# likojack/ODAM

Measured on AMD Instinct MI355X. Metric: frames/sec end-to-end (DETR detect + SQ fit), 640x480 ScanNet, 1/2/4/8 GPU, higher is better.
Workload: dtype f32

## Files before the change

include/odam_detr.h:

```cpp
#ifndef ODAM_DETR_H
#define ODAM_DETR_H
#ifdef __cplusplus
extern "C" {
#endif

typedef struct odam_detr odam_detr;

typedef struct {
    int resnet_blocks[4];
    int hidden_dim;
    int nheads;
    int dim_feedforward;
    int enc_layers;
    int dec_layers;
    int num_queries;
    int num_classes1;
    int angle_bins;
    int max_batch;
    int img_h, img_w;
    int dtype;
    int pre_norm;
    int dilation;
    int basic_block;
} odam_detr_cfg;
// ... 35 lines not shown
int odam_op_conv2d_nhwc(const float* x, const float* w_packed, const float* scale, const float* bias,
                        const float* residual, float* y, int B, int H, int W, int Cin, int Cout, int KH, int KW,
                        int stride, int pad, int Kpad, int relu, int k_order, void* stream);
int odam_op_conv2d_nhwc_bf16(const void* x, const void* w_packed, const float* scale, const float* bias,
                             const void* residual, void* y, int B, int H, int W, int Cin, int Cout, int KH, int KW,
                             int stride, int pad, int Kpad, int relu, int out_f32, int k_order, void* stream);
int odam_op_conv2d_nhwc_ex(const void* x, const void* w_packed, const float* scale, const float* bias, const void* residual,
                           void* y, int B, int H, int W, int Cin, int Cout, int KH, int KW, int stride, int pad, int dil,
                           int Kpad, int relu, int k_order, int dtype, int out_f32, void* stream);
int odam_op_bottleneck_bf16(const void* x, const void* w2, const float* s2, const float* b2, const void* w3, const float* s3,
                            const float* b3, const void* residual, void* y, const void* w1n, const float* s1n, const float* b1n,
                            void* y_next, int B, int H, int W, int P, int stride, int PN, void* stream);
int odam_op_bottleneck_f32(const float* x, const float* w2, const float* s2, const float* b2, const float* w3, const float* s3,
                           const float* b3, const float* residual, float* y, const float* w1n, const float* s1n, const float* b1n,
                           float* y_next, int B, int H, int W, int P, int stride, int PN, void* stream);
long long odam_op_conv_paths(char* buf, int n, int reset);
int odam_op_conv_bf16_mode(int mode);
int odam_op_conv_f32_mode(int mode);
long long odam_op_pooled_stem_launches(void);
int odam_op_attention(const float* Q, int ldq, const float* K, int ldk, const float* V, int ldv, float* O, int ldo,
                      int B, int H, int Lq, int Lk, void* stream);
int odam_op_attention_bf16(const void* Q, int ldq, const void* K, int ldk, const void* V, int ldv, void* O, int ldo,
                           int B, int H, int Lq, int Lk, void* stream);
int odam_op_add_layernorm(const float* x, const float* r, const float* gamma, const float* beta, float* y, int M,
                          void* stream);
int odam_op_attention_ex(const void* Q, int ldq, const void* K, int ldk, const void* V, int ldv, void* O, int ldo,
                         int B, int H, int Lq, int Lk, int head_dim, int dtype, const unsigned char* key_mask, void* stream);
int odam_op_add_layernorm_ex(const void* x, const void* r, const float* gamma, const float* beta, void* y,
                             const float* pos, int L, void* y_pos, int M, int dtype, void* stream);
int odam_op_quantize_mxfp8(const void* x, int src_dtype, long long n, void* q, void* s, void* stream);
int odam_op_dequantize_mxfp8(const void* q, const void* s, long long n, float* y, void* stream);
int odam_op_conv2d_nhwc_mxfp8(const void* x, const void* xs, const void* w_packed, const void* ws, const float* scale,
                              const float* bias, const void* residual, void* y, void* ys, void* y_bf16, float* y_f32,
                              int B, int H, int W, int Cin, int Cout, int KH, int KW, int stride, int pad, int dil,
// ... 8 lines not shown
```

odam_amd/csrc/cg_big.hpp:

```cpp
#pragma once
#include "cg_common.hpp"
#include "cg_tails_f32.hpp"
#include "cg_tail_bf16.hpp"
#include "cg_launch.h"

namespace odam_cg {

constexpr int big_bm(int BN, int NTH) { return (NTH == 1024 && BN == 64) ? 512 : 256; }
constexpr int big_wm(int MODE, int BN, int NTH) {
    return NTH == 1024 ? (BN == 64 ? 16 : 4)
         : MODE >= 3 ? (BN == 256 ? ((MODE == 4 && CG_X16_WM8) ? 8 : 4) : 8) : (BN == 256 ? 2 : (BN == 128 ? 4 : 8));
}
#ifndef CG_DEEP_A
#define CG_DEEP_A 1
#endif

constexpr bool big_deep_a(int MODE, int BN, int NST, int NTH) { return CG_DEEP_A != 0 && MODE == 0 && BN == 256 && NST == 4 && NTH == 1024; }
template <int MODE, int BN, int NST, int NTH>
constexpr int big_lds_bytes() {
    const int bm = big_bm(BN, NTH);
    const int ring = NST * (MODE >= 3 ? bm * 64 + 96 * BN : (bm + BN) * 64);
    const int wm = big_wm(MODE, BN, NTH);
    const int wn = NTH / 64 / wm;
    const int slab = MODE == 4 ? (NTH / 64) * 16 * ((BN / wn > 128 ? 128 : BN / wn) + 4) * 4 : (NTH / 64) * 32 * (BN / wn) * 4;
    const int s1 = (MODE == 0 && NTH == 512) ? (BN == 256 ? 2 : (BN == 128 ? 3 : 4)) * (384 * 64 + 3 * BN * 64) : 0;
    const int m = ring > slab ? ring : slab;
    const int deep = big_deep_a(MODE, BN, NST, NTH) ? (6 + 4) * 256 * 64 : 0;
    const int m2 = m > s1 ? m : s1;
    return m2 > deep ? m2 : deep;
}

template <int MODE, int BN, int NST, int NTH = 512, int FUSE = 0>
__global__ __launch_bounds__(NTH, (NTH == 1024 ? 4 : 2)) void conv_gemm_big_kernel(ConvGemmArgs a) {
    static_assert(!FUSE || (FUSE <= 4 && (MODE == 3 || MODE == 4) && NTH == 512 && ((FUSE != 3 && BN == 64) || (FUSE == 3 && BN == 128))) ||
                      (FUSE >= 5 && FUSE <= 8 && MODE == 0 && NTH == 512 && NST == 4),
                  "fused layers: pre-split filters with 64-column tiles (FUSE 1, 2, 4) or 128-column tiles (FUSE 3); bf16 (FUSE 5 + "
                  "log2(PN / 32), 5 = no chained reduce)");
    static_assert(MODE == 0 || MODE == 2 || MODE == 3 || MODE == 4,
                  "bf16 operands, fp32 split, fp32 split with pre-split filters (3: 32x32x16 matrix instruction, 4: 16x16x32)");
    static_assert(MODE != 4 || FUSE <= 4, "the 16x16x32 schedule: its own epilogue, or the fp32 bottleneck tails");
    constexpr bool BF16 = MODE == 0;
    constexpr bool PRE = MODE == 3 || MODE == 4;
    constexpr bool X16 = MODE == 4;
    static_assert(!PRE || NTH == 512 || (X16 && NTH == 1024), "pre-split filters: eight-wave workgroups, or sixteen waves (16x16x32 loop)");
    static_assert(NTH != 1024 || (FUSE == 0 && ((BN == 64 && (X16 || BF16)) || (BN == 256 && BF16))), "sixteen waves: plain layers (512 x 64: bf16 or the 16x16x32 split loop; 256 x 256: bf16)");
    using T = typename std::conditional<BF16, unsigned short, float>::type;
    constexpr int EPC = BF16 ? 8 : 4;
    constexpr int BM = big_bm(BN, NTH), BKE = 4 * EPC;
    constexpr int KU = 2 * BKE;
    constexpr int NW = NTH / 64;
    constexpr int WM = big_wm(MODE, BN, NTH), WN = NW / WM;
    constexpr int TM = BM / WM / 32, TN = BN / WN / 32;
    constexpr int RPP = NTH / 4;
    constexpr int A_LD = BM / RPP, B_LD = (BN + RPP - 1) / RPP;
    constexpr int ROWB = 64;
// ... 450 lines not shown
            for (int i = 0; i < MI; i++)
#pragma unroll
                for (int j = 0; j < NJ; j++) asm volatile("" :: "v"(c16[i][j]));
#if CG_HACK & 2
#pragma unroll
            for (int i = 0; i < 8; i++) asm volatile("" :: "v"(hk_l[i]));
#endif
            return;
        }
#endif
        if constexpr (FUSE != 0 || POOLABLE) __syncthreads();
        if constexpr (FUSE == 1) { fused_second(a, c16, smem, lds_base, m0, wave, lane); return; }
        if constexpr (FUSE == 2) { fused_chain(a, c16, smem, lds_base, m0, wave, lane); return; }
        if constexpr (FUSE == 3) { fused_second128(a, c16, smem, lds_base, m0, wave, lane); return; }
        if constexpr (FUSE == 4) { fused_chain128(a, c16, smem, lds_base, m0, wave, lane); return; }
        if constexpr (POOLABLE) {
            if (a.pool) {
                constexpr int SLD = BN + 4;
                static_assert(BM * SLD * 4 <= NST * STAGE, "the pooling slab fits the ring");
                float* S = smem;
                float scv[NJ], biv[NJ];
#pragma unroll
                for (int j = 0; j < NJ; j++) {
                    const int n = j * 16 + r16;
                    scv[j] = a.scale ? a.scale[n] : 1.0f; biv[j] = a.bias ? a.bias[n] : 0.0f;
                }
#pragma unroll
                for (int mi = 0; mi < MI; mi++)
#pragma unroll
                    for (int r = 0; r < 4; r++) {
// ... 450 lines not shown
                    const int n = wn * (BN / WN) + j * 32 + l32;
                    const float sc = a.scale ? a.scale[n] : 1.0f, bi = a.bias ? a.bias[n] : 0.0f;
#pragma unroll
                    for (int r = 0; r < 16; r++) {
                        const int R = wm * (BM / WM) + i * 32 + (r & 3) + 8 * (r >> 2) + 4 * half;
                        float v = acc[i][j][r] * sc + bi;
                        v = bf2f(f2bf(v));
                        S[R * SLD + n] = (pool_row_ok(R) && v > 0.f) ? v : 0.f;
                    }
                }
            __syncthreads();
            pool_store(S);
            return;
        }
    }
    if constexpr (FUSE >= 5) {
        fused_bf16<BN, FUSE == 5 ? 0 : (32 << (FUSE - 5)), FUSE == 7 ? 2 : 3>(a, acc, smem, lds_base, m0, wm, wn, wave, lane);
        return;
    }
    static_assert(X16 || (WM * WN * 32 * (BN / WN) * 4 <= big_lds_bytes<MODE, BN, NST, NTH>() && NST * STAGE <= big_lds_bytes<MODE, BN, NST, NTH>()),
                  "ring and epilogue staging fit the dynamic LDS");
    if (ep2) epilogue2<BM, BN, WM, WN, TM, TN, BF16>(a, acc, smem, m0, n0, wm, wn, wave, lane);
    else epilogue<BM, BN, WM, WN, TM, TN, BF16>(a, acc, smem, big_lds_bytes<MODE, BN, NST, NTH>() / 4, m0, n0, wm, wn, wave, lane);
}

#define g_s1_window odam_cfg::get(odam_cfg::CG_S1)

template <int MODE, int BN, int NST, int NTH = 512>
static int launch_big(const ConvGemmArgs& a_in, hipStream_t stream) {
    ConvGemmArgs a = a_in;
    a.s1_window = (MODE == 0 && NTH == 512) ? g_s1_window : 0;
// ... 21 lines not shown
```

odam_amd/csrc/cg_fused_f32.hip:

```cpp
#include "cg_big.hpp"

#include <algorithm>

namespace odam_cg {

template <int MODE>
static int launch_big_fused_as(const ConvGemmArgs& a, hipStream_t stream) {
    static const bool attr_ok = [] {
        return hipFuncSetAttribute((const void*)conv_gemm_big_kernel<MODE, 64, 4, 512, 1>, hipFuncAttributeMaxDynamicSharedMemorySize, FUSE_LDS_BYTES) == hipSuccess &&
               hipFuncSetAttribute((const void*)conv_gemm_big_kernel<MODE, 64, 4, 512, 2>, hipFuncAttributeMaxDynamicSharedMemorySize, FUSE_LDS_BYTES) == hipSuccess &&
               hipFuncSetAttribute((const void*)conv_gemm_big_kernel<MODE, 128, 4, 512, 3>, hipFuncAttributeMaxDynamicSharedMemorySize, FUSE_LDS_BYTES) == hipSuccess &&
               hipFuncSetAttribute((const void*)conv_gemm_big_kernel<MODE, 64, 4, 512, 4>, hipFuncAttributeMaxDynamicSharedMemorySize, FUSE_LDS_BYTES) == hipSuccess;
    }();
    if (!attr_ok) return odam_fail(2, "conv_gemm: cannot raise the dynamic LDS limit");
    const int tiles = (a.M + 255) / 256;
    if (a.Cout == 128) hipLaunchKernelGGL((conv_gemm_big_kernel<MODE, 128, 4, 512, 3>), dim3(tiles), dim3(512), FUSE_LDS_BYTES, stream, a);
    else if (a.G_Wt3 && a.G_N == 128) hipLaunchKernelGGL((conv_gemm_big_kernel<MODE, 64, 4, 512, 4>), dim3(tiles), dim3(512), FUSE_LDS_BYTES, stream, a);
    else if (a.G_Wt3) hipLaunchKernelGGL((conv_gemm_big_kernel<MODE, 64, 4, 512, 2>), dim3(tiles), dim3(512), FUSE_LDS_BYTES, stream, a);
    else hipLaunchKernelGGL((conv_gemm_big_kernel<MODE, 64, 4, 512, 1>), dim3(tiles), dim3(512), FUSE_LDS_BYTES, stream, a);
    ODAM_HIP(hipGetLastError());
    return 0;
}
int launch_big_fused(const ConvGemmArgs& a, hipStream_t stream) {
    const int m16 = odam_cfg::get(odam_cfg::CG_MFMA16);
    const bool x16 = a.Kpad % 32 == 0 && (m16 >= 3 || (m16 == 2 && a.Cout == 128));
    note_path("f32.fused.m%d.%s", x16 ? 4 : 3, a.Cout == 128 ? "l2" : !a.G_Wt3 ? "l1" : a.G_N == 128 ? "chain128" : "chain64");
    const long img_rows = (long)a.Ho * a.Wo, img_bytes = img_rows * a.F_ldc * 4;
    const int group = (int)std::min<long>(a.B, (0x7fffffffL - 1) / img_bytes);
    if (group < 1) return odam_fail(1, "conv_gemm: fused bottleneck: one image's output exceeds 2 GiB");
    const long lda = a.lda > 0 ? a.lda : a.Cin;
    for (int b0 = 0; b0 < a.B; b0 += group) {
        ConvGemmArgs g = a;
        g.B = std::min(group, a.B - b0);
        g.M = (int)(g.B * img_rows);
        g.A = reinterpret_cast<const float*>(a.A) + (size_t)b0 * a.H * a.W * lda;
        if (a.F_res) g.F_res = a.F_res + (size_t)b0 * img_rows * a.F_ldc;
        g.F_C = a.F_C + (size_t)b0 * img_rows * a.F_ldc;
        if (a.G_C) g.G_C = a.G_C + (size_t)b0 * img_rows * a.G_N;
        const int rc = x16 ? launch_big_fused_as<4>(g, stream) : launch_big_fused_as<3>(g, stream);
        if (rc) return rc;
    }
    return 0;
}

}

#if CG_STAMP
extern "C" int odam_cg_tail_stamps(unsigned long long* out8, int reset) {
    if (out8 && hipMemcpyFromSymbol(out8, HIP_SYMBOL(odam_cg::g_tail_stamps), 8 * sizeof(unsigned long long)) != hipSuccess) return 2;
    if (reset) {
        unsigned long long z[8] = {0, 0, 0, 0, 0, 0, 0, 0};
// ... 6 lines not shown
```

odam_amd/csrc/cg_tails_f32.hpp:

```cpp
#pragma once
#include "cg_common.hpp"

namespace odam_cg {

template <class ACC>
__device__ __forceinline__ void fused_second(const ConvGemmArgs& a, ACC& acc, float* smem, unsigned lds_base,
                                             int m0, int wave, int lane) {
    typedef __bf16 bf16x8 __attribute__((ext_vector_type(8)));
    const int half = lane >> 5, l32 = lane & 31;
    const int wave_u = __builtin_amdgcn_readfirstlane(wave);
    const TailAffine t1(a.scale, a.bias, a.relu, a.Cout), tF(a.F_scale, a.F_bias, a.F_relu, a.F_ldc);
    float sc1[4], bi1[4];
    cols64_affine(acc, t1, 0, lane, sc1, bi1);
    {
        const unsigned long long pf = (unsigned long long)a.F_Wt3;
        const u32x4 rs = u32x4{(unsigned)pf, (unsigned)(pf >> 32) & 0xffffu, OOB_VOFF, 0x00020000u};
#pragma unroll
        for (int j = 0; j < 12; j++) {
            const int q = wave_u + 8 * j;
            const int sp = q >> 3, rb = q & 7, s_ = sp / 3, pl = sp - 3 * s_;
            const int row = rb * 32 + (lane >> 1);
            const unsigned vo = (unsigned)(row * 384 + s_ * 96 + pl * 32 + (((lane & 1) ^ ((lane >> 4) & 1)) * 16));
            lds_dma16(rs, lds_base + (unsigned)(q * 1024), vo, 0);
        }
// ... 229 lines not shown
    wave_sync();
#pragma unroll
    for (int it = 0; it < 8; it++) {
        const int row = it * 4 + (lane >> 4);
        const int m = m_base + row;
        const float4 v = *reinterpret_cast<const float4*>(&slab[row * 64 + ((c4 ^ (row & 15)) << 2)]);
        if (m < a.M) *reinterpret_cast<float4*>(a.G_C + (size_t)m * 64 + c4 * 4) = v;
    }
#if CG_STAMP
    CG_TSTAMP(7);
    if (lane == 0) {
        for (int i = 0; i < 8; i++) if (i != 5) atomicAdd(&g_tail_stamps[i], ts_acc[i]);
        atomicAdd(&g_tail_stamps[5], 1ull);
    }
#endif
}

template <class ACC>
__device__ __forceinline__ void fused_chain128(const ConvGemmArgs& a, ACC& acc, float* smem, unsigned lds_base,
                                               int m0, int wave, int lane) {
    typedef __bf16 bf16x8 __attribute__((ext_vector_type(8)));
    constexpr int SLABS = 8 * 32 * 64 * 4, GB = 4 * 3 * 64 * 32, GB2 = 4 * 3 * 128 * 32;
    static_assert(SLABS + 2 * GB + GB2 == 160 * 1024, "slabs, two expand groups and one reduce slice fill the LDS");
    int half = lane >> 5, l32 = lane & 31;
    const int wave_u = __builtin_amdgcn_readfirstlane(wave);
    const TailAffine t1(a.scale, a.bias, a.relu, a.Cout), tF(a.F_scale, a.F_bias, a.F_relu, a.F_ldc);
    float sc1[4], bi1[4];
    cols64_affine(acc, t1, 0, lane, sc1, bi1);
    const unsigned long long pf = (unsigned long long)a.F_Wt3, pg = (unsigned long long)a.G_Wt3;
    const u32x4 rsf = u32x4{(unsigned)pf, (unsigned)(pf >> 32) & 0xffffu, OOB_VOFF, 0x00020000u};
// ... 286 lines not shown
```

odam_amd/csrc/conv_gemm.h:

```cpp
#pragma once
#include <hip/hip_runtime.h>
#include <stdint.h>

namespace odam_cg {

constexpr int ODAM_CG_F32 = 0;
constexpr int ODAM_CG_BF16 = 1;

struct ConvGemmArgs {
    const void* A;
    const void* Wt;
    const void* Wt3 = nullptr;
    const float* scale;
    const float* bias;
    const void* res;
    void* C;
    int B, H, W, Cin, log2Cin;
    int Ho, Wo, Cout;
    int KH, KW, stride, pad;
    int Kpad;
    int relu;
    int M;
    int ldc;
    int dtype;
    int out_f32;
    int lda;
    int k_order;
    const void* F_Wt3 = nullptr;
    const float* F_scale = nullptr;
    const float* F_bias = nullptr;
    const float* F_res = nullptr;
    float* F_C = nullptr;
    int F_ldc = 0, F_relu = 0;
    const void* G_Wt3 = nullptr;
    const float* G_scale = nullptr;
    const float* G_bias = nullptr;
    float* G_C = nullptr;
    int G_N = 64;
    const void* F_Wt = nullptr;
    const void* G_Wt = nullptr;
    int dil = 1;
    int pool = 0, pool_ph = 0, pool_pw = 0, Hp = 0, Wp = 0;
    int no_pin = 0;
    int s1_window = 0;
};

constexpr int POOL_PH = 8, POOL_PW = 14;

int launch_conv_gemm(const ConvGemmArgs& a, hipStream_t stream);

void set_big_mode(int mode);

void set_f32_mode(int mode);
// ... 15 lines not shown
```

odam_amd/csrc/conv_gemm.hip:

```cpp
#include "conv_gemm.h"

#include "cg_common.hpp"
#include "cg_launch.h"

#include <algorithm>
#include <cstdarg>
#include <cstdio>
#include <mutex>

namespace odam_cg {

static std::mutex g_path_mu;
static char g_path_ring[PATH_LOG_N][PATH_TOKEN_LEN];
static long long g_path_head = 0, g_path_base = 0;

void note_path(const char* fmt, ...) {
    char tok[PATH_TOKEN_LEN];
    va_list ap;
    va_start(ap, fmt);
    vsnprintf(tok, sizeof(tok), fmt, ap);
    va_end(ap);
    std::lock_guard<std::mutex> lk(g_path_mu);
    memcpy(g_path_ring[g_path_head % PATH_LOG_N], tok, sizeof(tok));
    g_path_head++;
// ... 377 lines not shown
    const bool x3 = !bf && ut && g_big_f32 == 2 && odam_cfg::get(odam_cfg::CG_SMALL_X3) != 0;
    note_path("%s.small.%dx%d.w%d%s%s%s", bf ? "bf16" : "f32", BM, BN, WM * WN, ut ? ".ut" : "", x3 ? ".x3" : "", ut && NST_UT == 4 ? ".s4" : "");
    if (bf) {
        if (ut) hipLaunchKernelGGL((conv_gemm_kernel<BM, BN, WM, WN, true, true, NST_UT>), g, b, 0, stream, a);
        else hipLaunchKernelGGL((conv_gemm_kernel<BM, BN, WM, WN, true, false>), g, b, 0, stream, a);
    } else {
        if (x3)
            hipLaunchKernelGGL((conv_gemm_kernel<BM, BN, WM, WN, false, true, NST_UT, true>), g, b, 0, stream, a);
        else if (ut) hipLaunchKernelGGL((conv_gemm_kernel<BM, BN, WM, WN, false, true, NST_UT>), g, b, 0, stream, a);
        else hipLaunchKernelGGL((conv_gemm_kernel<BM, BN, WM, WN, false, false>), g, b, 0, stream, a);
    }
    ODAM_HIP(hipGetLastError());
    return 0;
}

bool fused_second_ok(const ConvGemmArgs& a) {
    const int fuse = odam_cfg::get(odam_cfg::CG_FUSE);
    if (!fuse || !g_big_mode || g_big_f32 != 2 || a.dtype != ODAM_CG_F32) return false;
    if (!a.F_Wt3 || !a.F_C || !a.Wt3 || a.Kpad % 16 != 0) return false;
    const bool l1 = a.Cout == 64 && a.F_ldc == 256, l2 = a.Cout == 128 && a.F_ldc == 512 && !a.G_Wt3;
    if ((!l1 && !l2) || a.dil != 1) return false;
    if ((long)a.Cout * a.Kpad * 6 >= 0x7fffffffL || (long)a.Ho * a.Wo * a.F_ldc * 4 >= 0x7fffffffL) return false;
    if (a.G_Wt3 && (fuse < 2 || !a.G_C || (a.G_N != 64 && a.G_N != 128))) return false;
    return big_eligible(a, a.Cout);
}

#define g_fuse_bf16 odam_cfg::get(odam_cfg::CG_FUSE_BF16)
bool fused_bf16_ok(const ConvGemmArgs& a) {
    if (!g_fuse_bf16 || !g_big_mode || a.dtype != ODAM_CG_BF16 || !a.F_Wt || !a.F_C) return false;
    if (a.Cout != 64 && a.Cout != 128 && a.Cout != 256) return false;
    if (a.F_ldc != 4 * a.Cout || a.KH * a.KW != 9 || a.Cin != a.Cout || !a.k_order || a.dil != 1) return false;
    if ((long)a.M * a.F_ldc * 2 >= 0x7fffffffL) return false;
    if (a.G_Wt) {
        if (g_fuse_bf16 < 2 || !a.G_C) return false;
        const bool built = (a.Cout == 64 && (a.G_N == 64 || a.G_N == 128)) || (a.Cout == 128 && a.G_N == 128);
        if (!built) return false;
    }
    return big_eligible(a, a.Cout);
// ... 76 lines not shown
```

odam_amd/csrc/detr_model.hip:

```cpp
#include <hip/hip_runtime.h>
#include <atomic>

#include <algorithm>
#include <cmath>
#include <cstdlib>
#include <cstring>
#include <map>
#include <string>
#include <vector>

#include "../../include/odam_detr.h"
#include "cg_mx8.h"
#include "conv_gemm.h"
#include "detr_kernels.h"
#include "odam_config.h"
#include "odam_err.h"

using odam_cg::ConvGemmArgs;

namespace {

struct HostTensor {
    std::vector<long long> shape;
    std::vector<float> data;
// ... 243 lines not shown
            hipEvent_t e;
            ODAM_HIP(hipEventCreate(&e));
            m->ev.push_back(e);
        }
        m->ev_flops.resize(m->ev.size() / 2);
    }
    const int Ho = conv_out(H, (c.KH - 1) * c.dil + 1, c.stride, c.pad), Wo = conv_out(W, (c.KW - 1) * c.dil + 1, c.stride, c.pad);
    const int Cin_true = (c.KH == 7) ? 3 : c.Cin;
    m->ev_flops[m->ev_used / 2] = 2.0 * B * Ho * Wo * (double)c.Cout * c.KH * c.KW * Cin_true;
    ODAM_HIP(hipEventRecord(m->ev[m->ev_used], st));
    int rc = run_conv(c, x, B, H, W, res, relu, y, 0, st, m->dt, out_f32);
    ODAM_HIP(hipEventRecord(m->ev[m->ev_used + 1], st));
    m->ev_used += 2;
    return rc;
}
int fused_c2c3_t(odam_detr* m, const Conv& c2, const Conv& c3, const void* x, int B, int H, int W, const void* res, void* y,
                 hipStream_t st, const Conv* next_c1 = nullptr, void* t_next = nullptr, bool* chained = nullptr) {
    if (chained) *chained = false;
    if (m->basic) return -1;
    if (c2.dil != 1) return -1;
    if (c3.KH != 1 || c3.stride != 1 || c3.Kpad != c2.Cout) return -1;
    if (!m->dt && (!c2.w3 || !c3.w3)) return -1;
    ConvGemmArgs a{};
    a.dtype = m->dt; a.out_f32 = 0;
    a.A = x; a.Wt = c2.w; a.Wt3 = c2.w3; a.scale = c2.scale; a.bias = c2.bias; a.res = nullptr; a.C = nullptr;
    a.B = B; a.H = H; a.W = W; a.Cin = c2.Cin; a.log2Cin = ilog2(c2.Cin);
    a.Ho = conv_out(H, c2.KH, c2.stride, c2.pad); a.Wo = conv_out(W, c2.KW, c2.stride, c2.pad);
    a.Cout = c2.Cout; a.KH = c2.KH; a.KW = c2.KW; a.stride = c2.stride; a.pad = c2.pad; a.Kpad = c2.Kpad;
    a.relu = 1; a.M = B * a.Ho * a.Wo; a.ldc = c2.Cout; a.k_order = c2.k_order;
    a.F_scale = c3.scale; a.F_bias = c3.bias; a.F_res = (const float*)res; a.F_C = (float*)y;
    a.F_ldc = c3.Cout; a.F_relu = 1;
    double flops3 = 0.0;
// ... 11 lines not shown
        }
        if (!odam_cg::fused_bf16_ok(a)) return -1;
    } else {
    a.F_Wt3 = c3.w3;
    if (next_ok && next_c1->w3 && (next_c1->Cout == 64 || next_c1->Cout == 128) && c3.Cout == 256) {
        a.G_Wt3 = next_c1->w3; a.G_scale = next_c1->scale; a.G_bias = next_c1->bias; a.G_C = (float*)t_next; a.G_N = next_c1->Cout;
        if (odam_cg::fused_second_ok(a)) {
            if (chained) *chained = true;
            flops3 = 2.0 * a.M * (double)next_c1->Cout * c3.Cout;
        } else {
            a.G_Wt3 = nullptr; a.G_scale = a.G_bias = nullptr; a.G_C = nullptr; a.G_N = 64;
        }
    }
    if (!odam_cg::fused_second_ok(a)) return -1;
    }
    if (!m->profile) return odam_cg::launch_conv_gemm(a, st);
    if (m->ev_used + 2 > m->ev.size()) {
        for (int k = 0; k < 2; k++) {
            hipEvent_t e;
            ODAM_HIP(hipEventCreate(&e));
            m->ev.push_back(e);
        }
        m->ev_flops.resize(m->ev.size() / 2);
    }
    m->ev_flops[m->ev_used / 2] = 2.0 * a.M * ((double)c2.Cout * c2.KH * c2.KW * c2.Cin + (double)c3.Cout * c2.Cout) + flops3;
    ODAM_HIP(hipEventRecord(m->ev[m->ev_used], st));
    int rc = odam_cg::launch_conv_gemm(a, st);
    ODAM_HIP(hipEventRecord(m->ev[m->ev_used + 1], st));
    m->ev_used += 2;
    return rc;
}

static std::atomic<long long> g_pooled_stem_launches{0};
int stem_rows_t(odam_detr* m, int B, hipStream_t st, void* pooled_out = nullptr, bool* pooled = nullptr) {
    const Conv& c = m->stem_rows;
    const odam_detr_cfg& g = m->cfg;
    ConvGemmArgs a{};
    a.dtype = m->dt; a.out_f32 = 0;
    a.A = m->x4; a.Wt = c.w; a.Wt3 = c.w3; a.scale = c.scale; a.bias = c.bias; a.res = nullptr; a.C = m->stem_out;
    a.B = B; a.H = g.img_h + 6; a.W = g.img_w + 8; a.Cin = 32; a.log2Cin = 5; a.lda = 4;
// ... 386 lines not shown
            RC(conv_t(m, b.ds, cur, B, H, W, nullptr, false, m->dsb, st));
            res = m->dsb;
        }
        RC(conv_t(m, b.c2, tin, B, Ho, Wo, res, true, nxt, st));
        char* t = cur; cur = nxt; nxt = t;
        H = Ho; W = Wo;
    }
    for (size_t i = 0; !m->mx && !m->basic && i < m->blocks.size(); i++) {
        mark(i);
        const Bottleneck& b = m->blocks[i];
        const int s = m->block_stride[i];
        const int Ho = conv_out(H, 3, s, 1), Wo = conv_out(W, 3, s, 1);
        if (!have_c1) RC(conv_t(m, b.c1, cur, B, H, W, nullptr, true, tin, st));
        have_c1 = false;
        const char* res = cur;
        if (b.has_ds) {
            RC(conv_t(m, b.ds, cur, B, H, W, nullptr, false, m->dsb, st));
            res = m->dsb;
        }
        const Conv* next_c1 = (i + 1 < m->blocks.size()) ? &m->blocks[i + 1].c1 : nullptr;
        bool chained = false;
        const int frc = fused_c2c3_t(m, b.c2, b.c3, tin, B, H, W, res, nxt, st, next_c1, tout, &chained);
        if (frc > 0) return frc;
        if (frc < 0) {
            RC(conv_t(m, b.c2, tin, B, H, W, nullptr, true, tout, st));
            RC(conv_t(m, b.c3, tout, B, Ho, Wo, res, true, nxt, st));
        } else if (chained) {
            char* t = tin; tin = tout; tout = t;
            have_c1 = true;
        }
        char* t = cur; cur = nxt; nxt = t;
        H = Ho; W = Wo;
    }
    m->layer4 = cur;
    m->stage_ev[5] = m->ev_used;
    const int L = m->L, M = B * L, Mq = B * Q;

    RC(conv_t(m, m->input_proj, cur, B, H, W, nullptr, false, m->src, st));
    const float* pos = pos_b ? pos_b : m->pos;
// ... 231 lines not shown
    if (!odam_cg::fused_second_ok(a)) return odam_fail(4, "odam_op_bottleneck_f32: the fused kernel does not apply to this shape");
    unsigned short *d2 = nullptr, *d3 = nullptr, *d1 = nullptr;
    int rc = split_filters_for_call(w2, P, 9 * P, st, &d2, "odam_op_bottleneck_f32");
    if (!rc) rc = split_filters_for_call(w3, 4 * P, P, st, &d3, "odam_op_bottleneck_f32");
    if (!rc && PN > 0) rc = split_filters_for_call(w1n, PN, 4 * P, st, &d1, "odam_op_bottleneck_f32");
    if (!rc) {
        a.Wt3 = d2; a.F_Wt3 = d3; a.G_Wt3 = PN > 0 ? d1 : nullptr;
        rc = odam_cg::launch_conv_gemm(a, st);
    }
    (void)hipStreamSynchronize(st);
    if (d2) (void)hipFree(d2);
    if (d3) (void)hipFree(d3);
    if (d1) (void)hipFree(d1);
    return rc;
}

extern "C" long long odam_op_conv_paths(char* buf, int n, int reset) { return odam_cg::read_paths(buf, n, reset); }

extern "C" int odam_op_conv_bf16_mode(int mode) {
    if (mode < 0 || mode > 2) return odam_fail(1, "odam_op_conv_bf16_mode: mode must be 0, 1 or 2");
    odam_cg::set_big_mode(mode);
    return 0;
}

extern "C" int odam_op_conv_f32_mode(int mode) {
    if (mode != 0 && mode != 2) return odam_fail(1, "odam_op_conv_f32_mode: mode must be 0 or 2");
    odam_cg::set_f32_mode(mode);
    return 0;
}

// ... 219 lines not shown
```

odam_amd/csrc/odam_common.hip:

```cpp
#include <atomic>
#include <cstdio>
#include <cstring>

#include "odam_config.h"
#include "odam_err.h"

extern "C" const char* odam_last_error(void) { return g_odam_err; }

namespace odam_cfg {
namespace {
struct Entry { const char* name; int def, lo, hi; };
const Entry TABLE[N_KEYS] = {
    {"cg.ring", 1, 0, 2},        {"cg.f32", 2, 0, 2},         {"cg.fuse", 2, 0, 2},       {"cg.fuse_bf16", 2, 0, 2},
    {"cg.s1", 1, 0, 1},          {"cg.ut", 1, 0, 1},          {"cg.tiles", 31, 0, 31},      {"cg.force", 0, 0, 3},
    {"cg.presplit", 1, 0, 1},    {"cg.mfma16", 3, 0, 3},      {"att.x3", 1, 0, 1},         {"att.bf16_mfma", 1, 0, 1}, {"stem.rows", 1, 0, 1},
    {"assoc.persist", 2, 0, 2},  {"sq.split", 32, 1, 32},     {"sq.split_wait", 3000, 0, 100000000}, {"sq.lanes", 0, 0, 64},
    {"stem.pool", 1, 0, 1},
    {"cg.pin", 0, 0, 1},
    {"cg.small_x3", 1, 0, 1},
    {"assoc.sk_fast", 1, 0, 3},
    {"assoc.hungarian", 0, 0, 1},
    {"assoc.merge", 1, 0, 1},
    {"sq.two_per_cu", 1, 0, 1},
};
std::atomic<int> g_val[N_KEYS];
std::atomic<bool> g_init{false};
void init() {
    if (g_init.load(std::memory_order_acquire)) return;
    for (int k = 0; k < N_KEYS; k++) g_val[k].store(TABLE[k].def, std::memory_order_relaxed);
    g_init.store(true, std::memory_order_release);
}
}
int get(Key k) { init(); return g_val[k].load(std::memory_order_relaxed); }
void set(Key k, int v) { init(); g_val[k].store(v, std::memory_order_relaxed); }
}

extern "C" int odam_config_set(const char* key, int value) {
    using namespace odam_cfg;
// ... 37 lines not shown
```

odam_amd/csrc/odam_config.h:

```cpp
#pragma once

namespace odam_cfg {
enum Key {
    CG_RING,
    CG_F32,
    CG_FUSE,
    CG_FUSE_BF16,
    CG_S1,
    CG_UT,
    CG_TILES,
    CG_FORCE,
    CG_PRESPLIT,
    CG_MFMA16,
    ATT_X3,
    ATT_BF16_MFMA,
    STEM_ROWS,
    ASSOC_PERSIST,
    SQ_SPLIT,
    SQ_SPLIT_WAIT,
    SQ_LANES,
    STEM_POOL,
    CG_PIN,
    CG_SMALL_X3,
    ASSOC_SK_FAST,
    ASSOC_HUNGARIAN,
    ASSOC_MERGE,
    SQ_TWO_PER_CU,
    N_KEYS
};
int get(Key k);
void set(Key k, int v);
}
```

Before: 1149.

## Fold the bottleneck downsample 1x1 conv into the fused c2/c3 tile kernel

Adds a FUSE=9 variant of the fp32 pre-split 16x16x32 conv-GEMM that computes the downsample 1x1 projection of the block input on the same tile and uses it as the residual for the c3 epilogue. This drops a separate downsample launch and the write/read of the dsb intermediate for the first block of layer1 (stride 1, 64 channels). It adds LDS pressure, extra MFMA work per tile and more register use, and falls back to the old path when the shape or config does not fit. The new path is controlled by the cg.fuse_ds key, which is on by default.

```diff
diff --git a/include/odam_detr.h b/include/odam_detr.h
--- a/include/odam_detr.h
+++ b/include/odam_detr.h
@@ -73,10 +73,15 @@
 int odam_op_bottleneck_f32(const float* x, const float* w2, const float* s2, const float* b2, const float* w3, const float* s3,
                            const float* b3, const float* residual, float* y, const float* w1n, const float* s1n, const float* b1n,
                            float* y_next, int B, int H, int W, int P, int stride, int PN, void* stream);
+int odam_op_bottleneck_ds_f32(const float* x, const float* w2, const float* s2, const float* b2, const float* w3, const float* s3,
+                              const float* b3, const float* xin, const float* wd, const float* sd, const float* bd, float* y,
+                              const float* w1n, const float* s1n, const float* b1n, float* y_next, int B, int H, int W, int P,
+                              int stride, int PN, void* stream);
 long long odam_op_conv_paths(char* buf, int n, int reset);
 int odam_op_conv_bf16_mode(int mode);
 int odam_op_conv_f32_mode(int mode);
 long long odam_op_pooled_stem_launches(void);
+long long odam_op_fused_ds_launches(void);
 int odam_op_attention(const float* Q, int ldq, const float* K, int ldk, const float* V, int ldv, float* O, int ldo,
                       int B, int H, int Lq, int Lk, void* stream);
 int odam_op_attention_bf16(const void* Q, int ldq, const void* K, int ldk, const void* V, int ldv, void* O, int ldo,
diff --git a/odam_amd/csrc/cg_big.hpp b/odam_amd/csrc/cg_big.hpp
--- a/odam_amd/csrc/cg_big.hpp
+++ b/odam_amd/csrc/cg_big.hpp
@@ -33,12 +33,12 @@
 template <int MODE, int BN, int NST, int NTH = 512, int FUSE = 0>
 __global__ __launch_bounds__(NTH, (NTH == 1024 ? 4 : 2)) void conv_gemm_big_kernel(ConvGemmArgs a) {
     static_assert(!FUSE || (FUSE <= 4 && (MODE == 3 || MODE == 4) && NTH == 512 && ((FUSE != 3 && BN == 64) || (FUSE == 3 && BN == 128))) ||
-                      (FUSE >= 5 && FUSE <= 8 && MODE == 0 && NTH == 512 && NST == 4),
+                      (FUSE >= 5 && FUSE <= 8 && MODE == 0 && NTH == 512 && NST == 4) || (FUSE == 9 && MODE == 4 && NTH == 512 && BN == 64),
                   "fused layers: pre-split filters with 64-column tiles (FUSE 1, 2, 4) or 128-column tiles (FUSE 3); bf16 (FUSE 5 + "
-                  "log2(PN / 32), 5 = no chained reduce)");
+                  "log2(PN / 32), 5 = no chained reduce); FUSE 9 = FUSE 2 with the downsample on the tile (16x16x32 loop)");
     static_assert(MODE == 0 || MODE == 2 || MODE == 3 || MODE == 4,
                   "bf16 operands, fp32 split, fp32 split with pre-split filters (3: 32x32x16 matrix instruction, 4: 16x16x32)");
-    static_assert(MODE != 4 || FUSE <= 4, "the 16x16x32 schedule: its own epilogue, or the fp32 bottleneck tails");
+    static_assert(MODE != 4 || FUSE <= 4 || FUSE == 9, "the 16x16x32 schedule: its own epilogue, or the fp32 bottleneck tails");
     constexpr bool BF16 = MODE == 0;
     constexpr bool PRE = MODE == 3 || MODE == 4;
     constexpr bool X16 = MODE == 4;
@@ -519,6 +519,7 @@
         if constexpr (FUSE == 2) { fused_chain(a, c16, smem, lds_base, m0, wave, lane); return; }
         if constexpr (FUSE == 3) { fused_second128(a, c16, smem, lds_base, m0, wave, lane); return; }
         if constexpr (FUSE == 4) { fused_chain128(a, c16, smem, lds_base, m0, wave, lane); return; }
+        if constexpr (FUSE == 9) { fused_chain_ds(a, c16, smem, lds_base, m0, wave, lane); return; }
         if constexpr (POOLABLE) {
             if (a.pool) {
                 constexpr int SLD = BN + 4;
@@ -999,7 +1000,7 @@
             return;
         }
     }
-    if constexpr (FUSE >= 5) {
+    if constexpr (FUSE >= 5 && FUSE <= 8) {
         fused_bf16<BN, FUSE == 5 ? 0 : (32 << (FUSE - 5)), FUSE == 7 ? 2 : 3>(a, acc, smem, lds_base, m0, wm, wn, wave, lane);
         return;
     }
diff --git a/odam_amd/csrc/cg_fused_f32.hip b/odam_amd/csrc/cg_fused_f32.hip
--- a/odam_amd/csrc/cg_fused_f32.hip
+++ b/odam_amd/csrc/cg_fused_f32.hip
@@ -10,11 +10,15 @@
         return hipFuncSetAttribute((const void*)conv_gemm_big_kernel<MODE, 64, 4, 512, 1>, hipFuncAttributeMaxDynamicSharedMemorySize, FUSE_LDS_BYTES) == hipSuccess &&
                hipFuncSetAttribute((const void*)conv_gemm_big_kernel<MODE, 64, 4, 512, 2>, hipFuncAttributeMaxDynamicSharedMemorySize, FUSE_LDS_BYTES) == hipSuccess &&
                hipFuncSetAttribute((const void*)conv_gemm_big_kernel<MODE, 128, 4, 512, 3>, hipFuncAttributeMaxDynamicSharedMemorySize, FUSE_LDS_BYTES) == hipSuccess &&
-               hipFuncSetAttribute((const void*)conv_gemm_big_kernel<MODE, 64, 4, 512, 4>, hipFuncAttributeMaxDynamicSharedMemorySize, FUSE_LDS_BYTES) == hipSuccess;
+               hipFuncSetAttribute((const void*)conv_gemm_big_kernel<MODE, 64, 4, 512, 4>, hipFuncAttributeMaxDynamicSharedMemorySize, FUSE_LDS_BYTES) == hipSuccess &&
+               (MODE != 4 || hipFuncSetAttribute((const void*)conv_gemm_big_kernel<4, 64, 4, 512, 9>, hipFuncAttributeMaxDynamicSharedMemorySize, FUSE_LDS_BYTES) == hipSuccess);
     }();
     if (!attr_ok) return odam_fail(2, "conv_gemm: cannot raise the dynamic LDS limit");
     const int tiles = (a.M + 255) / 256;
-    if (a.Cout == 128) hipLaunchKernelGGL((conv_gemm_big_kernel<MODE, 128, 4, 512, 3>), dim3(tiles), dim3(512), FUSE_LDS_BYTES, stream, a);
+    if (a.D_Wt3) {
+        if constexpr (MODE != 4) return odam_fail(1, "conv_gemm: the downsample on the tile needs the 16x16x32 loop");
+        else hipLaunchKernelGGL((conv_gemm_big_kernel<4, 64, 4, 512, 9>), dim3(tiles), dim3(512), FUSE_LDS_BYTES, stream, a);
+    } else if (a.Cout == 128) hipLaunchKernelGGL((conv_gemm_big_kernel<MODE, 128, 4, 512, 3>), dim3(tiles), dim3(512), FUSE_LDS_BYTES, stream, a);
     else if (a.G_Wt3 && a.G_N == 128) hipLaunchKernelGGL((conv_gemm_big_kernel<MODE, 64, 4, 512, 4>), dim3(tiles), dim3(512), FUSE_LDS_BYTES, stream, a);
     else if (a.G_Wt3) hipLaunchKernelGGL((conv_gemm_big_kernel<MODE, 64, 4, 512, 2>), dim3(tiles), dim3(512), FUSE_LDS_BYTES, stream, a);
     else hipLaunchKernelGGL((conv_gemm_big_kernel<MODE, 64, 4, 512, 1>), dim3(tiles), dim3(512), FUSE_LDS_BYTES, stream, a);
@@ -35,6 +39,7 @@
         g.M = (int)(g.B * img_rows);
         g.A = reinterpret_cast<const float*>(a.A) + (size_t)b0 * a.H * a.W * lda;
         if (a.F_res) g.F_res = a.F_res + (size_t)b0 * img_rows * a.F_ldc;
+        if (a.D_x) g.D_x = a.D_x + (size_t)b0 * img_rows * 64;
         g.F_C = a.F_C + (size_t)b0 * img_rows * a.F_ldc;
         if (a.G_C) g.G_C = a.G_C + (size_t)b0 * img_rows * a.G_N;
         const int rc = x16 ? launch_big_fused_as<4>(g, stream) : launch_big_fused_as<3>(g, stream);
diff --git a/odam_amd/csrc/cg_tails_f32.hpp b/odam_amd/csrc/cg_tails_f32.hpp
--- a/odam_amd/csrc/cg_tails_f32.hpp
+++ b/odam_amd/csrc/cg_tails_f32.hpp
@@ -267,6 +267,229 @@
         atomicAdd(&g_tail_stamps[5], 1ull);
     }
 #endif
+}
+
+template <class ACC>
+__device__ __forceinline__ void fused_chain_ds(const ConvGemmArgs& a, ACC& acc, float* smem, unsigned lds_base,
+                                               int m0, int wave, int lane) {
+    typedef __bf16 bf16x8 __attribute__((ext_vector_type(8)));
+    constexpr int SLABS = 8 * 32 * 64 * 4, GB = 4 * 3 * 64 * 32;
+    constexpr int F_AT = SLABS, G_AT = SLABS + 2 * GB, D_AT = SLABS + 3 * GB;
+    static_assert(SLABS + 4 * GB == 160 * 1024, "slabs, two expand groups, one reduce slice and one downsample slice fill the LDS");
+    int half = lane >> 5, l32 = lane & 31, r16 = lane & 15, kq = lane >> 4;
+    const int wave_u = __builtin_amdgcn_readfirstlane(wave);
+    const TailAffine t1(a.scale, a.bias, a.relu, a.Cout), tF(a.F_scale, a.F_bias, a.F_relu, a.F_ldc), tD(a.D_scale, a.D_bias, 0, a.F_ldc);
+    float sc1[4], bi1[4];
+    cols64_affine(acc, t1, 0, lane, sc1, bi1);
+    const unsigned long long pf = (unsigned long long)a.F_Wt3, pg = (unsigned long long)a.G_Wt3, pd = (unsigned long long)a.D_Wt3;
+    const u32x4 rsf = u32x4{(unsigned)pf, (unsigned)(pf >> 32) & 0xffffu, OOB_VOFF, 0x00020000u};
+    const u32x4 rsg = u32x4{(unsigned)pg, (unsigned)(pg >> 32) & 0xffffu, OOB_VOFF, 0x00020000u};
+    const u32x4 rsd = u32x4{(unsigned)pd, (unsigned)(pd >> 32) & 0xffffu, OOB_VOFF, 0x00020000u};
+    const int swz = ((lane & 1) ^ ((lane >> 4) & 1)) * 16;
+    auto piece = [&](int j, int& s_, int& pl, int& row) {
+        const int q = wave_u + 8 * j, sp = q >> 1;
+        s_ = sp / 3; pl = sp - 3 * s_; row = (q & 1) * 32 + (lane >> 1);
+        return q;
+    };
+    auto dma_expand = [&](int g) {
+#pragma unroll
+        for (int j = 0; j < 3; j++) {
+            int s_, pl, row;
+            const int q = piece(j, s_, pl, row);
+            lds_dma16(rsf, lds_base + (unsigned)(F_AT + (g & 1) * GB + q * 1024), (unsigned)((64 * g + row) * 384 + s_ * 96 + pl * 32 + swz), 0);
+        }
+    };
+    auto dma_reduce = [&](int g) {
+#pragma unroll
+        for (int j = 0; j < 3; j++) {
+            int s_, pl, row;
+            const int q = piece(j, s_, pl, row);
+            lds_dma16(rsg, lds_base + (unsigned)(G_AT + q * 1024), (unsigned)(row * (16 * 96) + (4 * g + s_) * 96 + pl * 32 + swz), 0);
+        }
+    };
+    auto dma_ds = [&](int g) {
+#pragma unroll
+        for (int j = 0; j < 3; j++) {
+            int s_, pl, row;
+            const int q = piece(j, s_, pl, row);
+            lds_dma16(rsd, lds_base + (unsigned)(D_AT + q * 1024), (unsigned)((64 * g + row) * 384 + s_ * 96 + pl * 32 + (lane & 1) * 16), 0);
+        }
+    };
+    const int c4 = lane & 15;
+    const int m_base = m0 + wave * 32;
+    const size_t out_bytes = (size_t)a.M * a.F_ldc * 4;
+    const __amdgpu_buffer_rsrc_t out_rs = __builtin_amdgcn_make_buffer_rsrc(a.F_C, 0, (int)out_bytes, 0x00020000);
+    const __amdgpu_buffer_rsrc_t x_rs = __builtin_amdgcn_make_buffer_rsrc(const_cast<float*>(a.D_x), 0, (int)((size_t)a.M * 64 * 4), 0x00020000);
+    const int m_lane = m_base + (lane >> 4);
+    const unsigned off_lane = (unsigned)m_lane * 1024u + (unsigned)(c4 * 16);
+    auto voff = [&](int it, int g) -> unsigned { return (m_lane + it * 4 < a.M) ? off_lane + (unsigned)(it * 4096 + g * 256) : OOB_VOFF; };
+    dma_expand(0);
+    dma_ds(0);
+    float4 xr[2][2][2];
+#pragma unroll
+    for (int mi = 0; mi < 2; mi++) {
+        const int m = m_base + 16 * mi + r16;
+#pragma unroll
+        for (int kb = 0; kb < 2; kb++) {
+            const unsigned vo = (unsigned)m * 256u + (unsigned)(kb * 128 + kq * 32);
+            xr[mi][kb][0] = __builtin_bit_cast(float4, __builtin_amdgcn_raw_buffer_load_b128(x_rs, m < a.M ? vo : OOB_VOFF, 0, 0));
+            xr[mi][kb][1] = __builtin_bit_cast(float4, __builtin_amdgcn_raw_buffer_load_b128(x_rs, m < a.M ? vo + 16u : OOB_VOFF, 0, 0));
+        }
+    }
+    float* slab = smem + wave * (32 * 64);
+    auto slab_at = [](int row, int col) { return row * 64 + ((((col >> 2) ^ (row & 15)) << 2) | (col & 3)); };
+    auto frags = [&](uint4 (&xh)[4], uint4 (&xm)[4], uint4 (&xl)[4]) {
+#pragma unroll
+        for (int s_ = 0; s_ < 4; s_++) {
+            const float4 c0 = *reinterpret_cast<const float4*>(&slab[slab_at(l32, 16 * s_ + 8 * half)]);
+            const float4 c1 = *reinterpret_cast<const float4*>(&slab[slab_at(l32, 16 * s_ + 8 * half + 4)]);
+            cg_split8(c0, c1, xh[s_], xm[s_], xl[s_]);
+        }
+    };
+    auto wave_sync = [] {
+        __builtin_amdgcn_fence(__ATOMIC_RELEASE, "wavefront");
+        __builtin_amdgcn_wave_barrier();
+        __builtin_amdgcn_fence(__ATOMIC_ACQUIRE, "wavefront");
+    };
+    acc_cols64(acc, 0, lane, [&](int row, int c64, int j, float x) { slab[slab_at(row, c64)] = t1.act(x * sc1[j] + bi1[j]); });
+    wave_sync();
+    uint4 ah[4], am[4], al[4];
+    frags(ah, am, al);
+    floatx16 acc3[2];
+#pragma unroll
+    for (int jc = 0; jc < 2; jc++)
+#pragma unroll
+        for (int r = 0; r < 16; r++) acc3[jc][r] = 0.0f;
+    const char* lds_c = reinterpret_cast<const char*>(smem);
+    const char* wg = lds_c + G_AT;
+    const char* wd = lds_c + D_AT + (kq >> 1) * 3 * 2048 + r16 * 32 + (kq & 1) * 16;
+#define ODAM_MM2(accv, x, y) accv = __builtin_amdgcn_mfma_f32_32x32x16_bf16(__builtin_bit_cast(bf16x8, x), __builtin_bit_cast(bf16x8, y), accv, 0, 0, 0)
+#define ODAM_MM16(accv, x, y) accv = __builtin_amdgcn_mfma_f32_16x16x32_bf16(__builtin_bit_cast(bf16x8, x), __builtin_bit_cast(bf16x8, y), accv, 0, 0, 0)
+    asm volatile("s_waitcnt vmcnt(0)" ::: "memory");
+#pragma unroll 1
+    for (int g = 0; g < 4; g++) {
+        asm volatile("" : "+v"(half), "+v"(l32), "+v"(r16), "+v"(kq));
+        if (g > 0) asm volatile("s_waitcnt vmcnt(8)" ::: "memory");
+        __syncthreads();
+        if (g + 1 < 4) dma_expand(g + 1);
+        dma_reduce(g);
+        const int b_off = l32 * 32 + ((half ^ ((l32 >> 3) & 1)) * 16);
+        const char* wf = lds_c + F_AT + (g & 1) * GB;
+        {
+            float sdv[4], bdv[4];
+#pragma unroll
+            for (int nj = 0; nj < 4; nj++) { sdv[nj] = tD.scale1(64 * g + 16 * nj + r16); bdv[nj] = tD.bias1(64 * g + 16 * nj + r16); }
+            floatx4 cd[2][4];
+#pragma unroll
+            for (int mi = 0; mi < 2; mi++)
+#pragma unroll
+                for (int nj = 0; nj < 4; nj++) cd[mi][nj] = floatx4{0.f, 0.f, 0.f, 0.f};
+#pragma unroll
+            for (int mi = 0; mi < 2; mi++)
+#pragma unroll
+                for (int kb = 0; kb < 2; kb++) {
+                    uint4 xh, xm, xl;
+                    cg_split8(xr[mi][kb][0], xr[mi][kb][1], xh, xm, xl);
+#pragma unroll
+                    for (int nj = 0; nj < 4; nj++) {
+                        const char* bp = wd + kb * 6 * 2048 + nj * 16 * 32;
+                        const uint4 bh = *reinterpret_cast<const uint4*>(bp), bm = *reinterpret_cast<const uint4*>(bp + 2048),
+                                    bl = *reinterpret_cast<const uint4*>(bp + 4096);
+                        ODAM_MM16(cd[mi][nj], xl, bh); ODAM_MM16(cd[mi][nj], xm, bm); ODAM_MM16(cd[mi][nj], xh, bl);
+                        ODAM_MM16(cd[mi][nj], xm, bh); ODAM_MM16(cd[mi][nj], xh, bm);
+                        ODAM_MM16(cd[mi][nj], xh, bh);
+                        __builtin_amdgcn_sched_barrier(0);
+                    }
+                }
+            __builtin_amdgcn_wave_barrier();
+#pragma unroll
+            for (int mi = 0; mi < 2; mi++)
+#pragma unroll
+                for (int nj = 0; nj < 4; nj++)
+#pragma unroll
+                    for (int r = 0; r < 4; r++) {
+                        float v = cd[mi][nj][r] * sdv[nj] + bdv[nj];
+                        v += 0.0f;
+                        slab[slab_at(16 * mi + 4 * kq + r, 16 * nj + r16)] = v;
+                    }
+        }
+        wave_sync();
+        float scj[2], bij[2];
+#pragma unroll
+        for (int jb = 0; jb < 2; jb++) { scj[jb] = tF.scale1(64 * g + 32 * jb + l32); bij[jb] = tF.bias1(64 * g + 32 * jb + l32); }
+        floatx16 acc2[2];
+#pragma unroll
+        for (int jb = 0; jb < 2; jb++) {
+#pragma unroll
+            for (int r = 0; r < 16; r++) acc2[jb][r] = 0.0f;
+#pragma unroll
+            for (int s_ = 0; s_ < 4; s_++) {
+                const char* bp = wf + (s_ * 3) * 2048 + jb * 1024 + b_off;
+                const uint4 bh = *reinterpret_cast<const uint4*>(bp), bm = *reinterpret_cast<const uint4*>(bp + 2048),
+                            bl = *reinterpret_cast<const uint4*>(bp + 4096);
+                ODAM_MM2(acc2[jb], al[s_], bh); ODAM_MM2(acc2[jb], am[s_], bm); ODAM_MM2(acc2[jb], ah[s_], bl);
+                ODAM_MM2(acc2[jb], am[s_], bh); ODAM_MM2(acc2[jb], ah[s_], bm);
+                ODAM_MM2(acc2[jb], ah[s_], bh);
+                __builtin_amdgcn_sched_barrier(0);
+            }
+        }
+        __builtin_amdgcn_wave_barrier();
+        asm volatile("" : "+v"(half), "+v"(l32));
+#pragma unroll
+        for (int jb = 0; jb < 2; jb++)
+#pragma unroll
+            for (int r = 0; r < 16; r++) {
+                float* sp_ = &slab[slab_at((r & 3) + 8 * (r >> 2) + 4 * half, jb * 32 + l32)];
+                *sp_ = tF.act(acc2[jb][r] * scj[jb] + bij[jb] + *sp_);
+            }
+        wave_sync();
+        asm volatile("s_waitcnt vmcnt(0)" ::: "memory");
+        __syncthreads();
+        if (g + 1 < 4) dma_ds(g + 1);
+        asm volatile("" : "+v"(half), "+v"(l32));
+#pragma unroll
+        for (int it = 0; it < 8; it++) {
+            const int row = it * 4 + (lane >> 4);
+            const float4 o = *reinterpret_cast<const float4*>(&slab[row * 64 + ((c4 ^ (row & 15)) << 2)]);
+            __builtin_amdgcn_raw_buffer_store_b128(__builtin_bit_cast(u32x4, o), out_rs, voff(it, g), 0, 0);
+        }
+        uint4 xh[4], xm[4], xl[4];
+        frags(xh, xm, xl);
+#pragma unroll
+        for (int jc = 0; jc < 2; jc++)
+#pragma unroll
+            for (int s_ = 0; s_ < 4; s_++) {
+                const char* bp = wg + (s_ * 3) * 2048 + jc * 1024 + b_off;
+                const uint4 bh = *reinterpret_cast<const uint4*>(bp), bm = *reinterpret_cast<const uint4*>(bp + 2048),
+                            bl = *reinterpret_cast<const uint4*>(bp + 4096);
+                ODAM_MM2(acc3[jc], xl[s_], bh); ODAM_MM2(acc3[jc], xm[s_], bm); ODAM_MM2(acc3[jc], xh[s_], bl);
+                ODAM_MM2(acc3[jc], xm[s_], bh); ODAM_MM2(acc3[jc], xh[s_], bm);
+                ODAM_MM2(acc3[jc], xh[s_], bh);
+                __builtin_amdgcn_sched_barrier(0);
+            }
+        __builtin_amdgcn_wave_barrier();
+    }
+#undef ODAM_MM2
+#undef ODAM_MM16
+#pragma unroll
+    for (int jc = 0; jc < 2; jc++) {
+        const int n = jc * 32 + l32;
+        const float sc = a.G_scale ? a.G_scale[n] : 1.0f, bi = a.G_bias ? a.G_bias[n] : 0.0f;
+#pragma unroll
+        for (int r = 0; r < 16; r++) {
+            float v = acc3[jc][r] * sc + bi;
+            v = v > 0.f ? v : 0.f;
+            slab[slab_at((r & 3) + 8 * (r >> 2) + 4 * half, n)] = v;
+        }
+    }
+    wave_sync();
+#pragma unroll
+    for (int it = 0; it < 8; it++) {
+        const int row = it * 4 + (lane >> 4);
+        const int m = m_base + row;
+        const float4 v = *reinterpret_cast<const float4*>(&slab[row * 64 + ((c4 ^ (row & 15)) << 2)]);
+        if (m < a.M) *reinterpret_cast<float4*>(a.G_C + (size_t)m * 64 + c4 * 4) = v;
+    }
 }
 
 template <class ACC>
diff --git a/odam_amd/csrc/conv_gemm.h b/odam_amd/csrc/conv_gemm.h
--- a/odam_amd/csrc/conv_gemm.h
+++ b/odam_amd/csrc/conv_gemm.h
@@ -37,6 +37,10 @@
     const float* G_bias = nullptr;
     float* G_C = nullptr;
     int G_N = 64;
+    const float* D_x = nullptr;
+    const void* D_Wt3 = nullptr;
+    const float* D_scale = nullptr;
+    const float* D_bias = nullptr;
     const void* F_Wt = nullptr;
     const void* G_Wt = nullptr;
     int dil = 1;
diff --git a/odam_amd/csrc/conv_gemm.hip b/odam_amd/csrc/conv_gemm.hip
--- a/odam_amd/csrc/conv_gemm.hip
+++ b/odam_amd/csrc/conv_gemm.hip
@@ -415,6 +415,19 @@
     return 0;
 }
 
+static bool fused_ds_ok(const ConvGemmArgs& a) {
+    if (odam_cfg::get(odam_cfg::CG_FUSE_DS) == 0 || odam_cfg::get(odam_cfg::CG_FUSE) < 2 || !a.D_x) return false;
+    if (a.Cout != 64 || a.F_ldc != 256 || !a.G_Wt3 || a.G_N != 64 || a.Kpad % 32 != 0) return false;
+    if (a.stride != 1 || a.KH != 3 || a.KW != 3 || a.pad != 1 || a.Ho != a.H || a.Wo != a.W) return false;
+    if (odam_cfg::get(odam_cfg::CG_MFMA16) < 3 || odam_cfg::get(odam_cfg::CG_PRESPLIT) == 0) return false;
+    if ((long)a.Ho * a.Wo * 64 * 4 >= 0x7fffffffL) return false;
+    ConvGemmArgs d{};
+    d.dtype = ODAM_CG_F32; d.Wt3 = a.D_Wt3;
+    d.B = a.B; d.H = a.Ho; d.W = a.Wo; d.Cin = 64; d.log2Cin = 6; d.Ho = a.Ho; d.Wo = a.Wo; d.Cout = 256;
+    d.KH = d.KW = d.stride = 1; d.pad = 0; d.Kpad = 64; d.M = a.M; d.ldc = 256; d.no_pin = a.no_pin;
+    return big_eligible(d, 256);
+}
+
 bool fused_second_ok(const ConvGemmArgs& a) {
     const int fuse = odam_cfg::get(odam_cfg::CG_FUSE);
     if (!fuse || !g_big_mode || g_big_f32 != 2 || a.dtype != ODAM_CG_F32) return false;
@@ -423,6 +436,7 @@
     if ((!l1 && !l2) || a.dil != 1) return false;
     if ((long)a.Cout * a.Kpad * 6 >= 0x7fffffffL || (long)a.Ho * a.Wo * a.F_ldc * 4 >= 0x7fffffffL) return false;
     if (a.G_Wt3 && (fuse < 2 || !a.G_C || (a.G_N != 64 && a.G_N != 128))) return false;
+    if (a.D_Wt3 && !fused_ds_ok(a)) return false;
     return big_eligible(a, a.Cout);
 }
 
diff --git a/odam_amd/csrc/detr_model.hip b/odam_amd/csrc/detr_model.hip
--- a/odam_amd/csrc/detr_model.hip
+++ b/odam_amd/csrc/detr_model.hip
@@ -281,8 +281,10 @@
     m->ev_used += 2;
     return rc;
 }
+static std::atomic<long long> g_fused_ds_launches{0};
 int fused_c2c3_t(odam_detr* m, const Conv& c2, const Conv& c3, const void* x, int B, int H, int W, const void* res, void* y,
-                 hipStream_t st, const Conv* next_c1 = nullptr, void* t_next = nullptr, bool* chained = nullptr) {
+                 hipStream_t st, const Conv* next_c1 = nullptr, void* t_next = nullptr, bool* chained = nullptr,
+                 const Conv* ds = nullptr, const void* ds_x = nullptr) {
     if (chained) *chained = false;
     if (m->basic) return -1;
     if (c2.dil != 1) return -1;
@@ -324,6 +326,20 @@
     }
     if (!odam_cg::fused_second_ok(a)) return -1;
     }
+    bool folded = false;
+    if (ds) {
+        if (!m->dt && ds->w3 && ds->KH == 1 && ds->stride == 1 && ds->Cin == 64 && ds->Kpad == 64 && ds->Cout == c3.Cout) {
+            a.D_x = (const float*)ds_x; a.D_Wt3 = ds->w3; a.D_scale = ds->scale; a.D_bias = ds->bias; a.F_res = nullptr;
+            folded = odam_cg::fused_second_ok(a);
+            if (!folded) { a.D_x = nullptr; a.D_Wt3 = nullptr; a.D_scale = a.D_bias = nullptr; }
+        }
+        if (!folded) {
+            RC(conv_t(m, *ds, ds_x, B, H, W, nullptr, false, m->dsb, st));
+            a.F_res = (const float*)m->dsb;
+        } else {
+            g_fused_ds_launches.fetch_add(1);
+        }
+    }
     if (!m->profile) return odam_cg::launch_conv_gemm(a, st);
     if (m->ev_used + 2 > m->ev.size()) {
         for (int k = 0; k < 2; k++) {
@@ -333,7 +349,8 @@
         }
         m->ev_flops.resize(m->ev.size() / 2);
     }
-    m->ev_flops[m->ev_used / 2] = 2.0 * a.M * ((double)c2.Cout * c2.KH * c2.KW * c2.Cin + (double)c3.Cout * c2.Cout) + flops3;
+    m->ev_flops[m->ev_used / 2] = 2.0 * a.M * ((double)c2.Cout * c2.KH * c2.KW * c2.Cin + (double)c3.Cout * c2.Cout) + flops3 +
+                                  (folded ? 2.0 * a.M * (double)ds->Cout * ds->Cin : 0.0);
     ODAM_HIP(hipEventRecord(m->ev[m->ev_used], st));
     int rc = odam_cg::launch_conv_gemm(a, st);
     ODAM_HIP(hipEventRecord(m->ev[m->ev_used + 1], st));
@@ -750,15 +767,15 @@
         if (!have_c1) RC(conv_t(m, b.c1, cur, B, H, W, nullptr, true, tin, st));
         have_c1 = false;
         const char* res = cur;
-        if (b.has_ds) {
-            RC(conv_t(m, b.ds, cur, B, H, W, nullptr, false, m->dsb, st));
-            res = m->dsb;
-        }
         const Conv* next_c1 = (i + 1 < m->blocks.size()) ? &m->blocks[i + 1].c1 : nullptr;
         bool chained = false;
-        const int frc = fused_c2c3_t(m, b.c2, b.c3, tin, B, H, W, res, nxt, st, next_c1, tout, &chained);
+        const int frc = fused_c2c3_t(m, b.c2, b.c3, tin, B, H, W, res, nxt, st, next_c1, tout, &chained, b.has_ds ? &b.ds : nullptr, cur);
         if (frc > 0) return frc;
         if (frc < 0) {
+            if (b.has_ds) {
+                RC(conv_t(m, b.ds, cur, B, H, W, nullptr, false, m->dsb, st));
+                res = m->dsb;
+            }
             RC(conv_t(m, b.c2, tin, B, H, W, nullptr, true, tout, st));
             RC(conv_t(m, b.c3, tout, B, Ho, Wo, res, true, nxt, st));
         } else if (chained) {
@@ -1020,6 +1037,44 @@
     if (d1) (void)hipFree(d1);
     return rc;
 }
+
+extern "C" int odam_op_bottleneck_ds_f32(const float* x, const float* w2, const float* s2, const float* b2, const float* w3,
+                                         const float* s3, const float* b3, const float* xin, const float* wd, const float* sd,
+                                         const float* bd, float* y, const float* w1n, const float* s1n, const float* b1n, float* y_next,
+                                         int B, int H, int W, int P, int stride, int PN, void* stream) {
+    if (!x || !w2 || !w3 || !xin || !wd || !y || !w1n || !y_next) return odam_fail(1, "odam_op_bottleneck_ds_f32: null pointer");
+    if (P != 64 || stride != 1 || PN != 64) return odam_fail(5, "odam_op_bottleneck_ds_f32: the fold is built for P = 64, stride 1, PN = 64");
+    hipStream_t st = (hipStream_t)stream;
+    ConvGemmArgs a{};
+    a.dtype = 0;
+    a.A = x; a.Wt = w2; a.scale = s2; a.bias = b2;
+    a.B = B; a.H = H; a.W = W; a.Cin = P; a.log2Cin = ilog2(P);
+    a.Ho = conv_out(H, 3, stride, 1); a.Wo = conv_out(W, 3, stride, 1);
+    a.Cout = P; a.KH = 3; a.KW = 3; a.stride = stride; a.pad = 1; a.Kpad = 9 * P;
+    a.relu = 1; a.M = B * a.Ho * a.Wo; a.ldc = P; a.k_order = 1;
+    a.F_scale = s3; a.F_bias = b3; a.F_C = y; a.F_ldc = 4 * P; a.F_relu = 1;
+    a.G_scale = s1n; a.G_bias = b1n; a.G_C = y_next; a.G_N = PN;
+    a.D_x = xin; a.D_scale = sd; a.D_bias = bd;
+    a.Wt3 = w2; a.F_Wt3 = w3; a.G_Wt3 = w1n; a.D_Wt3 = wd;
+    if (!odam_cg::fused_second_ok(a)) return odam_fail(5, "odam_op_bottleneck_ds_f32: the fold does not apply to this shape or configuration");
+    unsigned short *d2 = nullptr, *d3 = nullptr, *d1 = nullptr, *dd = nullptr;
+    int rc = split_filters_for_call(w2, P, 9 * P, st, &d2, "odam_op_bottleneck_ds_f32");
+    if (!rc) rc = split_filters_for_call(w3, 4 * P, P, st, &d3, "odam_op_bottleneck_ds_f32");
+    if (!rc) rc = split_filters_for_call(w1n, PN, 4 * P, st, &d1, "odam_op_bottleneck_ds_f32");
+    if (!rc) rc = split_filters_for_call(wd, 4 * P, P, st, &dd, "odam_op_bottleneck_ds_f32");
+    if (!rc) {
+        a.Wt3 = d2; a.F_Wt3 = d3; a.G_Wt3 = d1; a.D_Wt3 = dd;
+        rc = odam_cg::launch_conv_gemm(a, st);
+    }
+    (void)hipStreamSynchronize(st);
+    if (d2) (void)hipFree(d2);
+    if (d3) (void)hipFree(d3);
+    if (d1) (void)hipFree(d1);
+    if (dd) (void)hipFree(dd);
+    return rc;
+}
+
+extern "C" long long odam_op_fused_ds_launches(void) { return g_fused_ds_launches.load(); }
 
 extern "C" long long odam_op_conv_paths(char* buf, int n, int reset) { return odam_cg::read_paths(buf, n, reset); }
 
diff --git a/odam_amd/csrc/odam_common.hip b/odam_amd/csrc/odam_common.hip
--- a/odam_amd/csrc/odam_common.hip
+++ b/odam_amd/csrc/odam_common.hip
@@ -22,6 +22,7 @@
     {"assoc.hungarian", 0, 0, 1},
     {"assoc.merge", 1, 0, 1},
     {"sq.two_per_cu", 1, 0, 1},
+    {"cg.fuse_ds", 1, 0, 1},
 };
 std::atomic<int> g_val[N_KEYS];
 std::atomic<bool> g_init{false};
diff --git a/odam_amd/csrc/odam_config.h b/odam_amd/csrc/odam_config.h
--- a/odam_amd/csrc/odam_config.h
+++ b/odam_amd/csrc/odam_config.h
@@ -26,6 +26,7 @@
     ASSOC_HUNGARIAN,
     ASSOC_MERGE,
     SQ_TWO_PER_CU,
+    CG_FUSE_DS,
     N_KEYS
 };
 int get(Key k);
```

Result: no change. 1155 (median of 6 runs) (+0.6%).
